# Anony-CFFM/CFFM

Measured on AMD Instinct MI355X. Metric: training examples/sec, frappe 10-field dim32; embedding-gather %HBM roofline, higher is better.
Workload: dtype f32; 1 GPU; frappe shape: synthetic libfm, 10 fields, 5382 features, inner/outer dim 32, batch 256 per GPU, selu, Adagrad lr 0.05, square_loss (README.md:28); global_batch=256, id_distribution=uniform, tables=replicated, parallelism=single

## Files before the change

### cffm_amd/csrc/common.hpp

```cpp
#pragma once
#include <hip/hip_runtime.h>
#include <stdint.h>

#include "../../include/cffm_hip.h"

#define CFFM_WAVE 64

#ifdef CFFM_PHASE_TIMERS
static __device__ unsigned long long cffm_phase_times[16];
static __device__ unsigned long long cffm_wg_times[2 * 1024];
static __device__ unsigned long long cffm_bwd_times[48];
#define PHASE_MARKB(i, wg) do { if ((wg) == 7 && threadIdx.x == 0) cffm_bwd_times[i] = wall_clock64(); } while (0)
#define PHASE_MARK(i) do { if (blockIdx.x == 7 && threadIdx.x == 0) cffm_phase_times[i] = wall_clock64(); } while (0)
#define PHASE_MARK2(i) do {} while (0)
#define PHASE_MARK3(i) do { if (CL && blockIdx.x == 7 && threadIdx.x == 0) cffm_phase_times[8 + (i)] = wall_clock64(); } while (0)
#else
#define PHASE_MARK(i) do {} while (0)
#define PHASE_MARK2(i) do {} while (0)
#define PHASE_MARK3(i) do {} while (0)
#define PHASE_MARKB(i, wg) do {} while (0)
#endif

typedef float f32x4 __attribute__((ext_vector_type(4)));
__device__ __forceinline__ int fused_c_off(int l, int c0, int c1, int D, int Pp) {
// ... 255 lines not shown

__device__ __forceinline__ float act_pos(float c, int act) {
    switch (act) {
        case CFFM_ACT_SELU: return CFFM_SELU_SCALE * c;
        case CFFM_ACT_GELU: return c * (0.5f * (1.f + erff(c * 0.70710678118654752440f)));
        default: return c;
    }
}

__device__ __forceinline__ float act_relu_grad(float c, int act) {
    return c > 0.f ? act_grad_f(c, act) : 0.f;
}

__device__ __forceinline__ void lds_barrier() {
    __builtin_amdgcn_fence(__ATOMIC_RELEASE, "workgroup", "local");
    __builtin_amdgcn_s_barrier();
    __builtin_amdgcn_fence(__ATOMIC_ACQUIRE, "workgroup", "local");
}

template <int CTRL, int ROW_MASK>
__device__ __forceinline__ float dpp_mov(float v, float identity) {
    return __builtin_bit_cast(float, __builtin_amdgcn_update_dpp(__builtin_bit_cast(int, identity), __builtin_bit_cast(int, v),
                                                                 CTRL, ROW_MASK, 0xf, false));
}
__device__ __forceinline__ float wave_sum(float v) {
    v += dpp_mov<0xB1, 0xf>(v, 0.f);
    v += dpp_mov<0x4E, 0xf>(v, 0.f);
    v += dpp_mov<0x141, 0xf>(v, 0.f);
    v += dpp_mov<0x140, 0xf>(v, 0.f);
    v += dpp_mov<0x142, 0xa>(v, 0.f);
    v += dpp_mov<0x143, 0xc>(v, 0.f);
    return __builtin_bit_cast(float, __builtin_amdgcn_readlane(__builtin_bit_cast(int, v), 63));
}
__device__ __forceinline__ float wave_max(float v) {
    const float ninf = -INFINITY;
    v = fmaxf(v, dpp_mov<0xB1, 0xf>(v, ninf));
    v = fmaxf(v, dpp_mov<0x4E, 0xf>(v, ninf));
    v = fmaxf(v, dpp_mov<0x141, 0xf>(v, ninf));
    v = fmaxf(v, dpp_mov<0x140, 0xf>(v, ninf));
    v = fmaxf(v, dpp_mov<0x142, 0xa>(v, ninf));
    v = fmaxf(v, dpp_mov<0x143, 0xc>(v, ninf));
    return __builtin_bit_cast(float, __builtin_amdgcn_readlane(__builtin_bit_cast(int, v), 63));
}

template <bool SIXTEEN>
__device__ __forceinline__ float row_group_sum(float v) {
    v += dpp_mov<0xB1, 0xf>(v, 0.f);
    v += dpp_mov<0x4E, 0xf>(v, 0.f);
    v += dpp_mov<0x141, 0xf>(v, 0.f);
    if (SIXTEEN) v += dpp_mov<0x140, 0xf>(v, 0.f);
    return v;
}

__device__ __forceinline__ float block_sum(float v, float* red) {
    v = wave_sum(v);
    const int w = threadIdx.x >> 6, nw = blockDim.x >> 6;
    __syncthreads();
    if ((threadIdx.x & 63) == 0) red[w] = v;
    __syncthreads();
    float t = 0.f;
    for (int i = 0; i < nw; ++i) t += red[i];
    return t;
}

__device__ __forceinline__ void build_pair_lut(uint32_t* lut, int F, int Pp) {
    for (int i = threadIdx.x; i < F; i += blockDim.x) {
        int base = i * (2 * F - i - 1) / 2;
        for (int j = i + 1; j < F; ++j) lut[base + j - i - 1] = (uint32_t)i | ((uint32_t)j << 16);
    }
    const int P = F * (F - 1) / 2;
    for (int p = P + threadIdx.x; p < Pp; p += blockDim.x) lut[p] = 0u;
}

__device__ __forceinline__ int fast_div(int n, float inv_d) { return (int)(((float)n + 0.5f) * inv_d); }

__device__ __forceinline__ f32x4 mfma16(float a, float b, f32x4 c) {
    return __builtin_amdgcn_mfma_f32_16x16x4f32(a, b, c, 0, 0, 0);
}
```

### cffm_amd/csrc/conv.hip

```cpp
#include <cstdlib>
#include <cstring>

#include "internal.hpp"

#include <type_traits>

#include <stdlib.h>
#include "inner_body.hpp"
#include "head_body.hpp"
#include "sort_body.hpp"

#define KSTEP 32
#define WG_KM 64

__device__ __forceinline__ int64_t xcd_tile(int64_t per_xcd) {
    const int64_t id = blockIdx.x;
    return (id & 7) * per_xcd + (id >> 3);
}
__host__ __device__ static inline int64_t xcd_per(int64_t tiles) { return (tiles + 7) / 8; }

struct RowPos { int b, y, x; };
__device__ __forceinline__ RowPos row_pos(int64_t m, int lgSo) {
    RowPos p;
    const int So = 1 << lgSo;
// ... 1550 lines not shown
    int early_off, es_off;
};


__device__ __forceinline__ unsigned rank_key_id(int raw, int M) { return min((unsigned)raw, (unsigned)M); }
template <int NW, int F_ = 0>
__device__ __forceinline__ void rank_keys_body(const int32_t* __restrict__ ids, int n, int b, int F_rt, int M,
                                               unsigned long long* __restrict__ out, char* smem) {
    constexpr int MAXF = F_ ? F_ : RANK_MAXF;
    const int F = F_ ? F_ : F_rt;
    float* cnt = reinterpret_cast<float*>(smem);
    const int tid = threadIdx.x, lane = tid & 63, wave = tid >> 6;
    unsigned long long mine[MAXF];
#pragma unroll
    for (int f = 0; f < MAXF; ++f) {
        const int slot = b * F + (f < F ? f : 0);
        mine[f] = f < F ? (((unsigned long long)rank_key_id(ids[slot], M) << 32) | (unsigned)slot) : 0ull;
    }
    int c[MAXF];
#pragma unroll
    for (int f = 0; f < MAXF; ++f) c[f] = 0;
    constexpr int GRP = 8;
    for (int j0 = tid; j0 < n; j0 += 64 * NW * GRP) {
        unsigned idj[GRP];
#pragma unroll
        for (int u = 0; u < GRP; ++u) {
            const int j = j0 + 64 * NW * u;
            idj[u] = rank_key_id(ids[j < n ? j : n - 1], M);
        }
#pragma unroll
        for (int u = 0; u < GRP; ++u) {
            const int j = j0 + 64 * NW * u;
            const unsigned long long kj = j < n ? (((unsigned long long)idj[u] << 32) | (unsigned)j) : ~0ull;
#pragma unroll
            for (int f = 0; f < MAXF; ++f) c[f] += kj < mine[f] ? 1 : 0;
        }
    }
#pragma unroll
    for (int f = 0; f < MAXF; ++f) {
        const float t = wave_sum((float)c[f]);
        if (lane == 0) cnt[wave * RANK_MAXF + f] = t;
    }
    __syncthreads();
    if (tid < F) {
        float c = cnt[tid];
#pragma unroll
        for (int w = 1; w < NW; ++w) c += cnt[w * RANK_MAXF + tid];
        const int rank = (int)c;
        const int slot = b * F + tid;
        out[rank] = ((unsigned long long)rank_key_id(ids[slot], M) << 32) | (unsigned)slot;
    }
    __syncthreads();
}

template <int N, int NTH>
struct ParkFilter {
    float4 w[N];
    float4* dst;
    int n4;
    __device__ __forceinline__ void fetch(const float4* src, float4* dst_, int n4_) {
        dst = dst_; n4 = src != nullptr ? n4_ : 0;
#pragma unroll
        for (int ii = 0; ii < N; ++ii) {
            const int i = threadIdx.x + NTH * ii;
            w[ii] = i < n4 ? src[i] : make_float4(0.f, 0.f, 0.f, 0.f);
        }
    }
    __device__ __forceinline__ void operator()() const {
#pragma unroll
        for (int ii = 0; ii < N; ++ii) {
            const int i = threadIdx.x + NTH * ii;
            if (i < n4) dst[i] = w[ii];
        }
    }
};

template <int N> using IntC = std::integral_constant<int, N>;
#define CV(x) decltype(x)::value
template <int L0, int L1, class Fn>
__device__ __forceinline__ void static_for(Fn&& fn) {
    if constexpr (L0 < L1) { fn(IntC<L0>()); static_for<L0 + 1, L1>(fn); }
}

template <int NT, int G, int ACT, int LGSO = -1>
__device__ __forceinline__ void fused_layer_fwd(const ConvArgs& ca, int b, char* smem, const float* inL, float* outL) {
    const int lgSo = LGSO >= 0 ? LGSO : ca.lgSo;
    const int64_t rows = 1ll << (2 * lgSo), m_lo = (int64_t)b * rows, m_hi = m_lo + rows;
    if (rows >= 64) {
        for (int64_t m0 = m_lo; m0 < m_hi; m0 += 64) {
            if (m0 > m_lo) lds_barrier();
            conv_fwd_taps_body<NT, 4 / G, false, G, ACT, LGSO>(ca, m0, m_hi, smem, inL, outL, m_lo);
        }
    } else if (rows >= 32) {
        conv_fwd_taps_body<NT, (G >= 2 ? 1 : 2), false, G, ACT, LGSO>(ca, m_lo, m_hi, smem, inL, outL, m_lo);
    } else {
        conv_fwd_taps_body<NT, 1, false, G, ACT, LGSO>(ca, m_lo, m_hi, smem, inL, outL, m_lo);
    }
}

template <int NT, int NW, int ACT = -1, int F_ = 0, int K_ = 0, int D_ = 0>
__global__ __launch_bounds__(64 * NW) void fwd_all_kernel(FwdAllArgs fa) {
    constexpr int G = NW / 4, PP = NT * 16;
    constexpr bool CS = F_ != 0;
    constexpr FwdAllLds PL = fwd_all_lds_plan(CS ? F_ : 2, CS ? K_ : 4, CS ? D_ : 4, PP);
    static_assert(!CS || (F_ * (F_ - 1) / 2 + 15) / 16 * 16 == PP, "NT is the column tile count of F_ fields");
    static_assert(!CS || (PL.c0_off >= 0 && PL.early_fits), "the compiled shape keeps its activations in LDS and gathers early");
    extern __shared__ __attribute__((aligned(16))) char smem[];
    const int c0_off = CS ? PL.c0_off : fa.c0_off, c1_off = CS ? PL.c1_off : fa.c1_off, es_off = CS ? PL.es_off : fa.es_off;
    const int D = CS ? D_ : fa.inner.g.D;
    int live = fa.live;
    if (CS) { live = -1; for (int d = D_; d > 1; d >>= 1) ++live; }
    auto CL = [&](int l) -> float* {
        return c0_off >= 0 ? reinterpret_cast<float*>(smem + fused_c_off(l, c0_off, c1_off, D, PP)) : nullptr;
    };
    const bool lds_act = c0_off >= 0;
#ifdef CFFM_PHASE_TIMERS
    if (threadIdx.x == 0) cffm_wg_times[2 * blockIdx.x] = wall_clock64();
#endif
    auto example = [&](int b) __attribute__((always_inline)) {
        ParkFilter<(4 * PP * PP / 4 + 64 * NW - 1) / (64 * NW), 64 * NW> park;
        const bool early = fa.early_off > 0;
        park.fetch(early ? reinterpret_cast<const float4*>(fa.conv[0].W) : nullptr, reinterpret_cast<float4*>(smem), 4 * PP * PP / 4);
        char* smem_i = smem + (CS ? (early ? PL.t_off : 0) : fa.early_off);
        if (fa.rank_keys) rank_keys_body<NW, F_>(fa.ids, fa.n_rows, b, fa.inner.g.F, fa.inner.g.M, fa.keys_sorted, smem_i);
        PHASE_MARK(0);
        inner_fwd_body<ACT, decltype(park), F_, K_, D_>(fa.inner, b, smem_i, early ? reinterpret_cast<float*>(smem + es_off) : nullptr,
                                                        D + 1, park);
        if (lds_act) lds_barrier(); else __syncthreads();
// ... 5 lines not shown
                lds_barrier();
                PHASE_MARK(1 + l);
                fused_layer_fwd<NT, G, ACT, LGSO>(fa.conv[l], b, smem, CL(l - 1), CL(l));
            });
        } else {
            for (int l = 1; l < live; ++l) {
                if (lds_act) lds_barrier(); else __syncthreads();
                PHASE_MARK(1 + l);
                fused_layer_fwd<NT, G, ACT>(fa.conv[l], b, smem, CL(l - 1), CL(l));
            }
        }
        if (lds_act) lds_barrier(); else __syncthreads();
        PHASE_MARK(1 + live);
        head_fwd_body<NW, ACT, false, F_, D_>(fa.head, b, smem, lds_act, c0_off, c1_off);
        PHASE_MARK(2 + live);
    };
    if constexpr (CS) {
        static_assert(!CS || 4096 / (CS ? F_ : 1) <= 2 * 256, "two passes over a grid of 256 workgroups cover every accepted B");
        if ((int)blockIdx.x < fa.B) example((int)blockIdx.x);
        if (const int b = blockIdx.x + gridDim.x; b < fa.B) {
            __syncthreads();
            example(b);
        }
    } else {
        for (int b = blockIdx.x; b < fa.B; b += gridDim.x) {
            if (b != (int)blockIdx.x) __syncthreads();
            example(b);
        }
    }
#ifdef CFFM_PHASE_TIMERS
    if (threadIdx.x == 0) cffm_wg_times[2 * blockIdx.x + 1] = wall_clock64();
#endif
}

template <int NT, int F_, int D_, int NW, bool ONE = false>
__device__ __forceinline__ void conv0_fact_bwd_body(const DgradArgs& a, float* __restrict__ slabW, float* __restrict__ slabB,
                                                    int64_t slab_stride, char* smem, int wg, int nwg) {
    constexpr int PP = NT * 16, S = 16, NTH = 64 * NW, XQ = 16 / NW;
    const int F = F_ ? F_ : a.F, D = D_ ? D_ : a.D, Dp = D + 1, P = F_ ? F_ * (F_ - 1) / 2 : a.P, F2 = 2 * F;
    const int TP = S * PP + 16;
    float* Wl = reinterpret_cast<float*>(smem);
    float* T = Wl + 4 * PP * PP;
    float* part = T + 2 * F * TP;
    float* dEi = part + NW * 16 * 32;
    float* dEj = dEi + 32 * 16;
    float* bred = dEj + 32 * 16;
    float* rs = bred + NW * PP;
    float* Es = rs + 2 * F;
    const int tid = threadIdx.x, lane = tid & 63, wave = tid >> 6, r = lane & 15, kk = lane >> 4;
    float* sw = slabW + (int64_t)wg * slab_stride;
    float* sb = slabB + (int64_t)wg * slab_stride;
    PHASE_MARKB(12, wg);
    {
        const float4* wsrc = reinterpret_cast<const float4*>(a.W);
        for (int i = tid; i < 4 * PP * PP / 4; i += NTH) reinterpret_cast<float4*>(Wl)[i] = wsrc[i];
        for (int e = tid; e < 4 * (PP - P) * PP; e += NTH) {
            const int tap = e / ((PP - P) * PP), o = e - tap * ((PP - P) * PP);
            sw[(tap * PP + P) * PP + o] = 0.f;
        }
    }
    bool first = true;
    float bacc[NT];
#pragma unroll
    for (int nt = 0; nt < NT; ++nt) bacc[nt] = 0.f;

    for (int b = wg; b < a.B; b += nwg) {
        __syncthreads();
        {
            const float* e = a.Cprev + (int64_t)b * F * D;
            const float invD = 1.f / (float)D;
            for (int i = tid; i < F * D; i += NTH) {
                const int f = fast_div(i, invD), d = i - f * D;
                Es[f * Dp + d] = e[i];
            }
        }
        __syncthreads();
        const float* dCb = a.dC + (int64_t)b * S * S * PP;
        PHASE_MARKB(13, wg);
        for (int u = wave; u < 2 * (F - 1); u += NW) {
            const int i = u % (F - 1), dh = u / (F - 1);
            const int nj = F - 1 - i, K = 2 * nj, base = i * (2 * F - i - 1) / 2;
            f32x4 acc[NT];
#pragma unroll
            for (int nt = 0; nt < NT; ++nt) acc[nt] = (f32x4){0.f, 0.f, 0.f, 0.f};
            for (int k0 = 0; k0 < K; k0 += 4) {
                const int k = k0 + kk;
                const bool ok = k < K;
                const int dw = (ok && k >= nj) ? 1 : 0, jj = ok ? k - dw * nj : 0;
                const float av = ok ? Es[(i + 1 + jj) * Dp + 2 * r + dw] : 0.f;
                const float* wr = Wl + ((dh * 2 + dw) * PP + base + jj) * PP + r;
#pragma unroll
                for (int nt = 0; nt < NT; ++nt) acc[nt] = mfma16(av, ok ? wr[nt * 16] : 0.f, acc[nt]);
            }
            float* tp = T + (dh * F + i) * TP + r;
#pragma unroll
            for (int nt = 0; nt < NT; ++nt)
#pragma unroll
                for (int j = 0; j < 4; ++j) tp[(kk * 4 + j) * PP + nt * 16] = acc[nt][j];
        }
        for (int e = tid; e < 2 * S * PP; e += NTH) {
            const int dh = e / (S * PP), o = e - dh * (S * PP);
            T[(dh * F + F - 1) * TP + o] = 0.f;
        }
        __syncthreads();
        PHASE_MARKB(14, wg);
        {
            f32x4 acc[2] = {(f32x4){0.f, 0.f, 0.f, 0.f}, (f32x4){0.f, 0.f, 0.f, 0.f}};
            float4 av[XQ][NT];
#pragma unroll
            for (int q4 = 0; q4 < XQ; ++q4)
#pragma unroll
                for (int h = 0; h < NT; ++h)
                    av[q4][h] = *reinterpret_cast<const float4*>(dCb + ((int64_t)r * S + wave + NW * q4) * PP + 16 * h + 4 * kk);
#pragma unroll
            for (int q4 = 0; q4 < XQ; ++q4) {
                const int x = wave + NW * q4;
#pragma unroll
                for (int h = 0; h < NT; ++h) {
                    float4 bv[2];
#pragma unroll
                    for (int ct = 0; ct < 2; ++ct) {
                        const int n = ct * 16 + r;
                        bv[ct] = n < F2 ? *reinterpret_cast<const float4*>(T + n * TP + x * PP + 16 * h + 4 * kk)
                                        : make_float4(0.f, 0.f, 0.f, 0.f);
                    }
#pragma unroll
                    for (int ct = 0; ct < 2; ++ct) {
// ... 421 lines not shown
    constexpr int PP = NT * 16, UNR = 4, NTH = 256 * HALVES;
    float* Bs = reinterpret_cast<float*>(smem);
    uint32_t* lut = reinterpret_cast<uint32_t*>(Bs + WGT_SUB * PP);
    float* Es = reinterpret_cast<float*>(lut + (GEN ? PP : 0));
    const int tid = tid_in >= 0 ? tid_in : (int)threadIdx.x, lane = tid & 63, wid = tid >> 6, tap = wid & 3, half = wid >> 2;
    const int r = lane & 15, kk = lane >> 4;
    const int So = 1 << a.lgSo, Sin = 2 * So, P = a.P, Dp = a.D + 1, S2 = So * So, dh = tap >> 1, dw = tap & 1;
    const int n_ex_max = GEN ? WGT_SUB / S2 + 2 : 0;
    f32x4* red = reinterpret_cast<f32x4*>(Es + (GEN ? (n_ex_max * a.F * Dp + 7) / 4 * 4 : 0));
    const int64_t rows_per_slab = ((a.Mtot + nslab - 1) / nslab + 3) / 4 * 4;
    const int64_t m_lo = m_lo_o >= 0 ? m_lo_o : slab * rows_per_slab;
    const int64_t m_hi = m_lo_o >= 0 ? m_hi_o : min(a.Mtot, m_lo + rows_per_slab);

    f32x4 acc[NT][NT];
#pragma unroll
    for (int i = 0; i < NT; ++i)
#pragma unroll
        for (int q = 0; q < NT; ++q) acc[i][q] = (f32x4){0.f, 0.f, 0.f, 0.f};
    float bs[NT];
#pragma unroll
    for (int q = 0; q < NT; ++q) bs[q] = 0.f;
    int fi[NT], fj[NT];
    if (GEN) {
        build_pair_lut(lut, a.F, PP);
        __syncthreads();
#pragma unroll
        for (int i = 0; i < NT; ++i) { const uint32_t ij = lut[i * 16 + r]; fi[i] = (ij & 0xffff) * Dp; fj[i] = (ij >> 16) * Dp; }
    }

    bool done_small = false;
    if constexpr (!GEN && HALVES == 1 && NT <= 4) {
        if (m_hi - m_lo <= 16 * UNR) {
            done_small = true;
            const int dbgw = (a.lgSo == 3 && m_lo_o < 0) ? slab : -1;
            PHASE_MARKB(32, dbgw);
            const int nrow = (int)max((int64_t)0, m_hi - m_lo), nk = (nrow + 3) / 4;
            float av[4][UNR][NT];
#pragma unroll
            for (int g = 0; g < 4; ++g)
                if (g * UNR < nk) {
#pragma unroll
                    for (int u = 0; u < UNR; ++u) {
                        int64_t m = m_lo + 4 * (g * UNR + u) + kk;
                        if (g * UNR + u >= nk || m >= a.Mtot) m = a.Mtot - 1;
                        const RowPos rp = row_pos(m, a.lgSo);
                        const float* arow = a.in + (((int64_t)rp.b * Sin + 2 * rp.y + dh) * Sin + 2 * rp.x + dw) * PP + r;
#pragma unroll
                        for (int i = 0; i < NT; ++i) av[g][u][i] = arow[16 * i];
                    }
                }
            __syncthreads();
            {
                const float4* src = reinterpret_cast<const float4*>(a.dC + m_lo * PP);
                for (int e = tid; e < nrow * (PP / 4); e += NTH) reinterpret_cast<float4*>(Bs)[e] = src[e];
                for (int e = nrow * (PP / 4) + tid; e < 4 * nk * (PP / 4); e += NTH)
                    reinterpret_cast<float4*>(Bs)[e] = make_float4(0.f, 0.f, 0.f, 0.f);
            }
            __syncthreads();
            PHASE_MARKB(33, dbgw);
#pragma unroll
            for (int g = 0; g < 4; ++g)
                if (g * UNR < nk) {
#pragma unroll
                    for (int u = 0; u < UNR; ++u)
                        if (g * UNR + u < nk) {
                            float bv[NT];
#pragma unroll
                            for (int q = 0; q < NT; ++q) bv[q] = Bs[(4 * (g * UNR + u) + kk) * PP + q * 16 + r];
#pragma unroll
                            for (int q = 0; q < NT; ++q) bs[q] += bv[q];
#pragma unroll
                            for (int i = 0; i < NT; ++i) {
                                const float x = act_pos(av[g][u][i], act);
#pragma unroll
                                for (int q = 0; q < NT; ++q) acc[i][q] = mfma16(x, bv[q], acc[i][q]);
                            }
                        }
                }
        }
    }
    PHASE_MARKB(34, (a.lgSo == 3 && m_lo_o < 0 && done_small) ? slab : -1);
    for (int64_t ms = m_lo; ms < m_hi && !done_small; ms += WGT_SUB) {
        const int nrow = (int)min((int64_t)WGT_SUB, m_hi - ms);
        const int b_lo = (int)(ms >> (2 * a.lgSo));
        __syncthreads();
        {
            const float4* src = reinterpret_cast<const float4*>(a.dC + ms * PP);
            for (int e = tid; e < nrow * (PP / 4); e += NTH) reinterpret_cast<float4*>(Bs)[e] = src[e];
            for (int e = nrow * (PP / 4) + tid; e < ((nrow + 3) / 4 * 4) * (PP / 4); e += NTH)
                reinterpret_cast<float4*>(Bs)[e] = make_float4(0.f, 0.f, 0.f, 0.f);
        }
        if (GEN) {
            const int b_hi = (int)((ms + nrow - 1) >> (2 * a.lgSo));
            stage_examples(Es, a.in, b_lo, b_hi - b_lo + 1, a.B, a.F, a.D, Dp);
        }
        __syncthreads();
        const int nk = (nrow + 3) / 4;
        int k0 = 0, k1 = nk;
        if (HALVES == 2) {
            const int mid = min(nk, ((nk + 1) / 2 + UNR - 1) / UNR * UNR);
            k0 = half == 0 ? 0 : mid;
            k1 = half == 0 ? mid : nk;
        }
        auto load_a = [&](int k, float (&av)[UNR][NT]) {
#pragma unroll
            for (int u = 0; u < UNR; ++u) {
                const int row = 4 * (k + u) + kk;
                int64_t m = ms + row;
                if (k + u >= k1 || m >= a.Mtot) m = a.Mtot - 1;
// ... 129 lines not shown

struct Conv01Args {
    DgradArgs d0;
    float *slabW0, *slabB0;
    int64_t stride0;
    DgradArgs d1;
    WgradArgs w1, w2, w3;
    int n2, n3;
};

template <int NT, int F_, int D_, int ACT>
__global__ __launch_bounds__(1024) void conv01_bwd_kernel(Conv01Args a) {
    extern __shared__ __attribute__((aligned(16))) char smem[];
    const int b = blockIdx.x, grp = __builtin_amdgcn_readfirstlane((int)(threadIdx.x >> 8)), ltid = threadIdx.x & 255;
    PHASE_MARKB(40, b);
    dgrad_taps_body<NT, 1, false, 4, ACT>(a.d1, b, smem, 0, -1, 4);
    PHASE_MARKB(41, b);
    {
        char* gsm = smem + (size_t)grp * (64 * NT * 16 * 4);
        const WgradArgs& w = grp == 0 ? a.w1 : (grp == 1 ? a.w2 : a.w3);
        const int nsl = grp == 0 ? (int)gridDim.x : (grp == 1 ? a.n2 : a.n3);
        const int slab = grp == 1 ? b - ((int)gridDim.x - a.n2) : b;
        const bool mine = grp < 3 && slab >= 0 && slab < nsl;
        int64_t m_lo = 0, m_hi = 0;
        if (mine) {
            const int64_t per = grp == 0 ? (1ll << (2 * w.lgSo)) : CFFM_TOP_SLAB_ROWS;
            m_lo = (int64_t)slab * per;
            m_hi = min(w.Mtot, m_lo + per);
            if (m_hi < m_lo) m_hi = m_lo;
        }
        wgrad_taps_body<NT, false, 1, ACT>(w, mine ? slab : 0, nsl, gsm, m_lo, m_hi, ltid, mine);
    }
    __syncthreads();
    PHASE_MARKB(42, b);
    conv0_fact_bwd_body<NT, F_, D_, 16, true>(a.d0, a.slabW0, a.slabB0, a.stride0, smem, b, (int)gridDim.x);
}

struct BwdTopArgs {
    HeadBwdArgs hb;
    DgradArgs d[2];
    WgradArgs w[2];
    int lgSo[2];
    int n_layers;
    int wgrad_here;
    InnerBwdArgs ib;
    int n_inner;
    int n_keys;
    const int32_t* rank_ids;
    unsigned long long* keys_sorted;
    int n_rows;
};

template <int NT, int ACT = -1>
__global__ __launch_bounds__(256) void bwd_top_kernel(BwdTopArgs a) {
    extern __shared__ __attribute__((aligned(16))) char smem[];
    __shared__ float dh1s[CFFM_HEAD_UNITS];
    __shared__ float dt1s[1024];
    __shared__ float red[4];
    const int bid = blockIdx.x;
#ifdef CFFM_PHASE_TIMERS
    if (threadIdx.x == 0) cffm_wg_times[2 * blockIdx.x] = wall_clock64();
#endif
    if (bid < a.n_inner) {
        PHASE_MARKB(36, bid);
        const float L = head_bwd_loss(a.hb, false, red);
        __syncthreads();
        PHASE_MARKB(37, bid);
        if (a.rank_ids != nullptr && a.n_keys == 0) {
            for (int b = bid; b < a.hb.B; b += a.n_inner) rank_keys_body<4>(a.rank_ids, a.n_rows, b, a.hb.g.F, a.hb.g.M, a.keys_sorted, smem);
        }
        PHASE_MARKB(38, bid);
        inner_bwd_body<ACT, true>(a.ib, bid, a.n_inner, smem, L);
        PHASE_MARKB(39, bid);
#ifdef CFFM_PHASE_TIMERS
        if (threadIdx.x == 0) cffm_wg_times[2 * blockIdx.x + 1] = wall_clock64();
#endif
        return;
    }
    if (bid < a.n_inner + a.n_keys) {
        for (int b = bid - a.n_inner; b < a.hb.B; b += a.n_keys) rank_keys_body<4>(a.rank_ids, a.n_rows, b, a.hb.g.F, a.hb.g.M, a.keys_sorted, smem);
#ifdef CFFM_PHASE_TIMERS
        if (threadIdx.x == 0) cffm_wg_times[2 * blockIdx.x + 1] = wall_clock64();
#endif
        return;
    }
    const int b = bid - a.n_inner - a.n_keys;
    PHASE_MARKB(0, b);
    HeadBwdState st;
    head_bwd_begin(a.hb, b, st);
    PHASE_MARKB(1, b);
    const float L = head_bwd_loss(a.hb, b == 0, red);
    PHASE_MARKB(2, b);
    if (b < a.hb.B)
        head_bwd_example<ACT>(a.hb, b, st, b, head_dout(a.hb.loss, a.hb.out[b], a.hb.y[b], 1.f / (float)a.hb.Bg, L), dh1s, dt1s);
    PHASE_MARKB(3, b);
    head_bwd_end(a.hb, b, st);
    PHASE_MARKB(4, b);
    for (int t = 0; t < a.n_layers; ++t) {
        __syncthreads();
        const int64_t rows = 1ll << (2 * a.lgSo[t]);
        const int64_t m_lo = (int64_t)b * rows, m_hi = b < a.hb.B ? m_lo + rows : m_lo;
        if (a.wgrad_here) wgrad_taps_body<NT, false, 1, ACT>(a.w[t], b, (int)gridDim.x - a.n_inner - a.n_keys, smem, m_lo, m_hi);
        PHASE_MARKB(5 + 2 * t, b);
        for (int64_t m0 = m_lo; m0 < m_hi; m0 += 16) dgrad_taps_body<NT, 1, false, 1, ACT>(a.d[t], 0, smem, m0, m_hi);
        PHASE_MARKB(6 + 2 * t, b);
    }
#ifdef CFFM_PHASE_TIMERS
    if (threadIdx.x == 0) cffm_wg_times[2 * blockIdx.x + 1] = wall_clock64();
#endif
}

template <int... Vs, class Go>
static int with_int(int v, Go&& go) {
    int rc = CFFM_ERR_UNSUPPORTED;
    (void)((v == Vs ? (rc = go(IntC<Vs>()), true) : false) || ...);
    return rc;
}
#define NT4 1, 2, 3, 4
#define NT68 6, 8
template <class... P, class... A>
static int launch(void (*kernel)(P...), dim3 grid, dim3 block, size_t lds, hipStream_t st, const A&... args) {
    int rc = set_lds(kernel, lds);
    if (rc) return rc;
    hipLaunchKernelGGL(kernel, grid, block, lds, st, args...);
    CFFM_CHECK_LAUNCH();
// ... 1498 lines not shown
```

### cffm_amd/csrc/head_body.hpp

```cpp
#pragma once
#include "common.hpp"

struct HeadArgs {
    Geo g;
    int B;
    const float* Eo;
    const float* fb;
    const float* inner_out;
    const float* C[CFFM_MAX_LAYERS];
    const float *d1_w, *d1_b, *d2_w, *d2_b, *att_W, *att_b, *lin_w, *lin_b, *bias;
    const float* y;
    float *t1, *h1, *att, *out, *sqerr;
    int loss, inner_conv, outer_conv;
    int s0_ready = 0;
    const float* pool[CFFM_MAX_LAYERS] = {};
    int pool_np[CFFM_MAX_LAYERS] = {};
};

__device__ __forceinline__ float loss_term(float out_raw, float y, int loss, float* out_eval) {
    switch (loss) {
        case CFFM_LOSS_MAE: *out_eval = out_raw; return fabsf(y - out_raw);
        case CFFM_LOSS_SQUARE_L2: *out_eval = out_raw; return 0.5f * (y - out_raw) * (y - out_raw);
        case CFFM_LOSS_LOG: {
            const float s = 1.f / (1.f + expf(-out_raw));
// ... 184 lines not shown
        out += o;
        out += sc[1];
        out += biasv;
        float ev = out;
        if (a.y) a.sqerr[b] = loss_term(out, yv, a.loss, &ev);
        else if (a.loss == CFFM_LOSS_LOG) ev = 1.f / (1.f + expf(-out));
        a.out[b] = ev;
    }
}

struct HeadBwdArgs {
    Geo g;
    int B;
    int64_t Bg;
    const float *fb, *t1, *h1, *att, *out, *y, *Ctop;
    const float *d1_w, *d2_w, *att_W, *lin_w;
    float* scalars;
    const float* sqerr;
    float* loss_out;
    float *dout, *dt1, *dfb, *dCtop;
    float *s_attW, *s_attb, *s_bias, *s_d1w, *s_d1b, *s_d2w, *s_d2b, *s_linw, *s_linb;
    int64_t stride_front, stride_back;
    int64_t front_len, back_len;
    int loss, outer_conv;
    int unscaled;
};

struct HeadBwdState {
    float g_d2w, g_d1b, g_d2b, g_bias, g_linw, g_linb, g_attb;
    bool first;
};

__device__ __forceinline__ void head_bwd_begin(const HeadBwdArgs& a, int slab, HeadBwdState& st) {
    const int tid = threadIdx.x;
    float* s_attW = a.s_attW + (int64_t)slab * a.stride_front;
    float* s_d1w = a.s_d1w + (int64_t)slab * a.stride_back;
    for (int64_t e = tid; e < a.front_len; e += 256) s_attW[e] = 0.f;
    for (int64_t e = tid; e < a.back_len; e += 256) s_d1w[e] = 0.f;
    st.g_d2w = st.g_d1b = st.g_d2b = st.g_bias = st.g_linw = st.g_linb = st.g_attb = 0.f;
    st.first = true;
    __syncthreads();
}

__device__ __forceinline__ float head_bwd_loss(const HeadBwdArgs& a, bool publisher, float* red) {
    const int tid = threadIdx.x;
    float sum = 0.f, hybrid_log = 0.f;
    if (a.loss == CFFM_LOSS_HYBRID) {
        float p_sq = 0.f, p_log = 0.f;
        for (int i = tid; i < a.B; i += 256) {
            const float o = a.out[i], yy = a.y[i];
            p_sq += 0.5f * (yy - o) * (yy - o);
            p_log -= yy * logf(o + 1e-7f) + (1.f - yy) * logf(1.f - o + 1e-7f);
        }
        sum = block_sum(p_sq, red);
        __syncthreads();
        hybrid_log = block_sum(p_log, red);
        __syncthreads();
    } else if (a.unscaled) {
        sum = 0.f;
    } else if (a.sqerr) {
        float part = 0.f;
        for (int i = tid; i < a.B; i += 256) part += a.sqerr[i];
        sum = block_sum(part, red);
        __syncthreads();
    } else {
        sum = a.scalars[3];
    }
    const float invB = 1.f / (float)a.Bg;
    float L;
    if (a.loss == CFFM_LOSS_SQUARE_RMSE) L = a.unscaled ? 1.f : sqrtf(sum * invB + 1e-10f);
    else if (a.loss == CFFM_LOSS_SQUARE_L2) L = sum;
    else if (a.loss == CFFM_LOSS_HYBRID) L = 0.5f * sum + 0.5f * hybrid_log * invB;
    else L = sum * invB;
    if (publisher && tid == 0) {
        a.scalars[1] = L;
        if (a.sqerr) { a.scalars[0] = sum; a.scalars[3] = sum; }
        if (a.loss_out) a.loss_out[0] = L;
    }
    return L;
}

template <int ACTC = -1>
__device__ __forceinline__ void head_bwd_example(const HeadBwdArgs& a, int slab, HeadBwdState& st, int b, float d,
                                                 float* dh1s, float* dt1s) {
    const Geo& g = a.g;
    const int tid = threadIdx.x, lane = tid & 63, wave = tid >> 6;
    const int t1w = 2 * g.D - 2;
    float* s_attW = a.s_attW + (int64_t)slab * a.stride_front;
    float* s_d1w = a.s_d1w + (int64_t)slab * a.stride_back;
    const bool first = st.first;
    int off_top = 0;
    for (int i = 0; i < g.live; ++i) off_top += g.D >> i;
    if (tid == 0) { a.dout[b] = d; st.g_bias += d; }
    __syncthreads();
    if (a.outer_conv) {
        const float dd = d * g.beta_outer;
        if (tid < CFFM_HEAD_UNITS) {
            const float v = dd * a.d2_w[tid];
            dh1s[tid] = v;
            st.g_d2w += a.h1[(int64_t)b * CFFM_HEAD_UNITS + tid] * dd;
            st.g_d1b += v;
        }
        if (tid == 0) st.g_d2b += dd;
        __syncthreads();
        for (int k = tid; k < t1w; k += 256) {
            float s = 0.f;
            for (int q = 0; q < CFFM_HEAD_UNITS; ++q) s += dh1s[q] * a.d1_w[k * CFFM_HEAD_UNITS + q];
            dt1s[k] = s;
            a.dt1[(int64_t)b * t1w + k] = s;
        }
        for (int e = tid; e < t1w * CFFM_HEAD_UNITS; e += 256) {
            const int k = e / CFFM_HEAD_UNITS, q = e % CFFM_HEAD_UNITS;
            const float v = a.t1[(int64_t)b * t1w + k] * dh1s[q];
            s_d1w[e] = first ? v : s_d1w[e] + v;
        }
        __syncthreads();
        const int ntop = 4 * g.Pp;
        for (int e = tid; e < ntop; e += 256) {
            const int yy = e / (2 * g.Pp);
            const int64_t idx = (int64_t)b * ntop + e;
            a.dCtop[idx] = dt1s[off_top + yy] * act_relu_grad(a.Ctop[idx], ACTC >= 0 ? ACTC : g.act);
        }
    }
    if (wave == 0) {
        const float fbv = lane < g.F ? a.fb[(int64_t)b * g.F + lane] : 0.f;
        if (g.linear_att) {
            const float at = lane < g.F ? a.att[(int64_t)b * g.F + lane] : 0.f;
            const float dg = lane < g.F ? d * a.lin_w[lane] : 0.f;
            const float da = dg * fbv;
            const float sda = wave_sum(da * at);
            const float dz = at * (da - sda) / g.lamda_att;
            float dfbv = dg * at;
            for (int gI = 0; gI < g.F; ++gI) {
                const float dzg = __shfl(dz, gI, 64);
                if (lane < g.F) {
                    dfbv += dzg * a.att_W[lane * g.F + gI];
                    const float v = fbv * dzg;
                    s_attW[lane * g.F + gI] = first ? v : s_attW[lane * g.F + gI] + v;
                }
            }
            if (lane < g.F) a.dfb[(int64_t)b * g.F + lane] = dfbv;
            st.g_linw += fbv * at * d;
            st.g_attb += dz;
            if (lane == 0) st.g_linb += d;
        } else if (lane < g.F) {
            a.dfb[(int64_t)b * g.F + lane] = d;
        }
    }
    st.first = false;
}

__device__ __forceinline__ void head_bwd_end(const HeadBwdArgs& a, int slab, const HeadBwdState& st) {
    const int tid = threadIdx.x;
    const int64_t sof = (int64_t)slab * a.stride_front, sob = (int64_t)slab * a.stride_back;
    if (tid < CFFM_HEAD_UNITS) {
        a.s_d2w[sob + tid] = st.g_d2w;
        a.s_d1b[sob + tid] = st.g_d1b;
    }
    if (tid < a.g.F) {
        a.s_linw[sob + tid] = st.g_linw;
        a.s_attb[sof + tid] = st.g_attb;
    }
    if (tid == 0) {
        a.s_d2b[sob] = st.g_d2b;
        a.s_bias[sof] = st.g_bias;
        a.s_linb[sob] = st.g_linb;
    }
}
```

### cffm_amd/csrc/inner_body.hpp

```cpp
#pragma once
#include "common.hpp"

struct InnerUnit {
    float x0, x1, I0, I1, z0, z1, s0, s1, eix, eiy, ejx, ejy;
    int i, j;
};

__device__ __forceinline__ InnerUnit inner_unit(const float* E, const uint32_t* lut, int p, int t, int K,
                                                const float* cw, const float* cb, int act) {
    InnerUnit u;
    const uint32_t ij = lut[p];
    u.i = ij & 0xffff; u.j = ij >> 16;
    const float2 ei = *reinterpret_cast<const float2*>(&E[u.i * K + 2 * t]);
    const float2 ej = *reinterpret_cast<const float2*>(&E[u.j * K + 2 * t]);
    u.eix = ei.x; u.eiy = ei.y; u.ejx = ej.x; u.ejy = ej.y;
    u.I0 = ei.x * ej.x; u.I1 = ei.y * ej.y;
    u.x0 = act_f(u.I0, act); u.x1 = act_f(u.I1, act);
    u.z0 = u.x0 * cw[0] + u.x1 * cw[2] + cb[0];
    u.z1 = u.x0 * cw[1] + u.x1 * cw[3] + cb[1];
    const float mp = fmaxf(u.x0, u.x1);
    u.s0 = act_pos(fmaxf(u.z0, 0.f), act) + mp;
    u.s1 = act_pos(fmaxf(u.z1, 0.f), act) + mp;
    return u;
}
// ... 57 lines not shown
                reinterpret_cast<float4*>(fg.Eo + (int64_t)b * g.F * g.D)[j] = v;
                if (EoL != nullptr) {
                    float* e = EoL + f * EoLp + 4 * c;
                    e[0] = v.x; e[1] = v.y; e[2] = v.z; e[3] = v.w;
                }
            }
        }
        if (threadIdx.x < g.F) {
            const int raw = idb[threadIdx.x];
            const int id = raw < 0 ? 0 : (raw >= fg.M ? fg.M - 1 : raw);
            const int64_t slot = (int64_t)b * g.F + threadIdx.x;
            fg.fb[slot] = fg.fbias[id];
            fg.keys[slot] = ((unsigned long long)(unsigned)((raw < 0 || raw >= fg.M) ? fg.M : raw) << 32) | (unsigned long long)slot;
        }
    } else {
        mid();
        const float4* src = reinterpret_cast<const float4*>(Ei + (int64_t)b * g.F * g.K);
        for (int i = threadIdx.x; i < FK4; i += blockDim.x) reinterpret_cast<float4*>(E)[i] = src[i];
    }
    build_pair_lut(lut, g.F, g.Pp);
    float cw[4] = {cw_g[0], cw_g[1], cw_g[2], cw_g[3]};
    float cb[2] = {cb_g[0], cb_g[1]};
    const int K2 = g.K / 2, units = g.P * K2;
    const float2* wd2 = reinterpret_cast<const float2*>(wd);
    const float2 w2_first = (int)threadIdx.x < units ? wd2[threadIdx.x] : make_float2(0.f, 0.f);
    __syncthreads();
    const float invK2 = 1.f / (float)K2;
    float part = 0.f;
    for (int u = threadIdx.x; u < units; u += blockDim.x) {
        const int p = fast_div(u, invK2), t = u - p * K2;
        const InnerUnit v = inner_unit(E, lut, p, t, g.K, cw, cb, act);
        const float2 w2 = u == (int)threadIdx.x ? w2_first : wd2[u];
        part += v.s0 * w2.x + v.s1 * w2.y;
    }
    const float tot = block_sum(part, red);
    if (threadIdx.x == 0) inner_out[b] = tot + bd[0];
}

struct InnerBwdArgs {
    Geo g;
    int B;
    const float *Ei, *dout, *cw, *cb, *wd;
    const float *out, *y;
    int loss;
    float invB;
    float* dEi;
    float *slab_cw, *slab_cb, *slab_dw, *slab_db;
    int64_t slab_stride;
    const int32_t* idx = nullptr;
    int idxM = 0;
    int idxStride = 0;
};

template <int ACTC = -1, bool ONE = false>
__device__ __forceinline__ void inner_bwd_body(const InnerBwdArgs& a, int slab, int nslab, char* smem, float L = 1.f) {
    const Geo& g = a.g;
    const int act = ACTC >= 0 ? ACTC : g.act;
    const int B = a.B;
    const float* __restrict__ Ei = a.Ei; const float* __restrict__ dout = a.dout;
    const float* __restrict__ cw_g = a.cw; const float* __restrict__ cb_g = a.cb; const float* __restrict__ wd = a.wd;
    float* __restrict__ dEi = a.dEi;
    float* __restrict__ slab_cw = a.slab_cw + slab * a.slab_stride; float* __restrict__ slab_cb = a.slab_cb + slab * a.slab_stride;
    float* __restrict__ slab_dw = a.slab_dw + slab * a.slab_stride; float* __restrict__ slab_db = a.slab_db + slab * a.slab_stride;
    const int FK = g.F * g.K;
    float* E = reinterpret_cast<float*>(smem);
    float* dE = E + FK;
    uint32_t* lut = reinterpret_cast<uint32_t*>(dE + 4 * FK);
    float* red = reinterpret_cast<float*>(lut + g.Pp);
    const int wave = threadIdx.x >> 6;
    build_pair_lut(lut, g.F, g.Pp);
    if (threadIdx.x < 8) slab_cw[threadIdx.x] = 0.f;
    if (threadIdx.x < 4) slab_db[threadIdx.x] = 0.f;
    float cw[4] = {cw_g[0], cw_g[1], cw_g[2], cw_g[3]};
    float cb[2] = {cb_g[0], cb_g[1]};
    const int K2 = g.K / 2, units = g.P * K2;
    const float invK2 = 1.f / (float)K2;
    float gcw[4] = {0.f, 0.f, 0.f, 0.f}, gcb[2] = {0.f, 0.f}, gdb = 0.f;
    constexpr int UPRE = 4;
    const float2* wd2 = reinterpret_cast<const float2*>(wd);
    float2 w2p[UPRE];
#pragma unroll
    for (int k = 0; k < UPRE; ++k) {
        const int u = threadIdx.x + k * blockDim.x;
        w2p[k] = u < units ? wd2[u] : make_float2(0.f, 0.f);
    }
    bool first = true;
    for (int b = slab; b < B; b += nslab) {
        const float db = dout ? dout[b] : head_dout(a.loss, a.out[b], a.y[b], a.invB, L);
        __syncthreads();
        if (a.idx == nullptr) {
            const float4* src = reinterpret_cast<const float4*>(Ei + (int64_t)b * FK);
            for (int i = threadIdx.x; i < FK / 4; i += blockDim.x) reinterpret_cast<float4*>(E)[i] = src[i];
        } else {
            const int K4 = g.K >> 2;
            const float invK4 = 1.f / (float)K4;
            for (int i = threadIdx.x; i < FK / 4; i += blockDim.x) {
                const int f = fast_div(i, invK4), c = i - f * K4;
                reinterpret_cast<float4*>(E)[i] =
                    reinterpret_cast<const float4*>(row_ptr(Ei, a.idx, a.idxM, (int64_t)b * g.F + f, g.K, a.idxStride))[c];
            }
        }
        for (int i = threadIdx.x; i < 4 * FK; i += blockDim.x) dE[i] = 0.f;
        __syncthreads();
        float* myE = dE + wave * FK;
        auto unit_step = [&](int u, float2 w2) {
            const int p = fast_div(u, invK2), t = u - p * K2;
            const InnerUnit v = inner_unit(E, lut, p, t, g.K, cw, cb, act);
            const int64_t wi = (int64_t)p * g.K + 2 * t;
            float2 acc2 = first ? make_float2(0.f, 0.f) : *reinterpret_cast<float2*>(&slab_dw[wi]);
            acc2.x += v.s0 * db; acc2.y += v.s1 * db;
            *reinterpret_cast<float2*>(&slab_dw[wi]) = acc2;
            const float ds0 = db * w2.x, ds1 = db * w2.y;
            const float dz0 = ds0 * act_relu_grad(fmaxf(v.z0, 0.f), act);
            const float dz1 = ds1 * act_relu_grad(fmaxf(v.z1, 0.f), act);
            gcw[0] += dz0 * v.x0; gcw[1] += dz1 * v.x0; gcw[2] += dz0 * v.x1; gcw[3] += dz1 * v.x1;
            gcb[0] += dz0; gcb[1] += dz1;
            const float dmp = ds0 + ds1;
            const bool firstmax = v.x0 >= v.x1;
            const float dx0 = dz0 * cw[0] + dz1 * cw[1] + (firstmax ? dmp : 0.f);
            const float dx1 = dz0 * cw[2] + dz1 * cw[3] + (firstmax ? 0.f : dmp);
            const float dI0 = dx0 * act_grad_f(v.I0, act), dI1 = dx1 * act_grad_f(v.I1, act);
            atomicAdd(&myE[v.i * g.K + 2 * t], dI0 * v.ejx);
            atomicAdd(&myE[v.i * g.K + 2 * t + 1], dI1 * v.ejy);
            atomicAdd(&myE[v.j * g.K + 2 * t], dI0 * v.eix);
            atomicAdd(&myE[v.j * g.K + 2 * t + 1], dI1 * v.eiy);
        };
#pragma unroll
        for (int k = 0; k < UPRE; ++k) {
            const int u = threadIdx.x + k * blockDim.x;
            if (u < units) unit_step(u, w2p[k]);
        }
        for (int u = threadIdx.x + UPRE * blockDim.x; u < units; u += blockDim.x) unit_step(u, wd2[u]);
        if (threadIdx.x == 0) gdb += db;
        __syncthreads();
        for (int i = threadIdx.x; i < FK; i += blockDim.x)
            dEi[(int64_t)b * FK + i] = ((dE[i] + dE[FK + i]) + dE[2 * FK + i]) + dE[3 * FK + i];
        first = false;
        if constexpr (ONE) break;
    }
    if (first) {
        for (int64_t i = threadIdx.x; i < (int64_t)g.P * g.K; i += blockDim.x) slab_dw[i] = 0.f;
    }
    float r[7] = {gcw[0], gcw[1], gcw[2], gcw[3], gcb[0], gcb[1], gdb};
#pragma unroll
    for (int q = 0; q < 7; ++q) r[q] = wave_sum(r[q]);
    __syncthreads();
    if ((threadIdx.x & 63) == 0) {
#pragma unroll
        for (int q = 0; q < 7; ++q) dE[wave * 8 + q] = r[q];
    }
    __syncthreads();
    if (threadIdx.x == 0) {
        const int nw = blockDim.x >> 6;
#pragma unroll
        for (int q = 0; q < 7; ++q) {
            float t = 0.f;
            for (int w = 0; w < nw; ++w) t += dE[w * 8 + q];
            r[q] = t;
        }
        for (int q = 0; q < 4; ++q) slab_cw[q] = r[q];
        slab_cb[0] = r[4]; slab_cb[1] = r[5];
        slab_db[0] = r[6];
    }
}
```

Measured before the change: 2.981 million examples/s.

## Issue global loads early in backward kernels to hide latency behind loss reduction

Inner backward now prefetches the embedding row, out/y scalars and zeroes dE before computing the block-wide loss, passing the loss computation as a callback so the loads overlap it. Several copy loops are restructured to issue batches of loads before stores (loads_first, ParkFilter), attention-weight reads are batched in groups of 12, blockDim is replaced by a compile-time 256, and bwd_top_kernel gets an occupancy hint. The rank-key computation is removed from this kernel path, which risks changing behaviour if it is not done elsewhere; extra registers from the unrolled loads could also reduce occupancy.

```diff
diff --git a/cffm_amd/csrc/common.hpp b/cffm_amd/csrc/common.hpp
--- a/cffm_amd/csrc/common.hpp
+++ b/cffm_amd/csrc/common.hpp
@@ -331,9 +331,10 @@
     return v;
 }
 
+template <int NTH = 0>
 __device__ __forceinline__ float block_sum(float v, float* red) {
     v = wave_sum(v);
-    const int w = threadIdx.x >> 6, nw = blockDim.x >> 6;
+    const int w = threadIdx.x >> 6, nw = NTH ? NTH >> 6 : (int)blockDim.x >> 6;
     __syncthreads();
     if ((threadIdx.x & 63) == 0) red[w] = v;
     __syncthreads();
@@ -342,13 +343,15 @@
     return t;
 }
 
+template <int NTH = 0>
 __device__ __forceinline__ void build_pair_lut(uint32_t* lut, int F, int Pp) {
-    for (int i = threadIdx.x; i < F; i += blockDim.x) {
+    const int nth = NTH ? NTH : (int)blockDim.x;
+    for (int i = threadIdx.x; i < F; i += nth) {
         int base = i * (2 * F - i - 1) / 2;
         for (int j = i + 1; j < F; ++j) lut[base + j - i - 1] = (uint32_t)i | ((uint32_t)j << 16);
     }
     const int P = F * (F - 1) / 2;
-    for (int p = P + threadIdx.x; p < Pp; p += blockDim.x) lut[p] = 0u;
+    for (int p = P + threadIdx.x; p < Pp; p += nth) lut[p] = 0u;
 }
 
 __device__ __forceinline__ int fast_div(int n, float inv_d) { return (int)(((float)n + 0.5f) * inv_d); }
@@ -356,3 +359,43 @@
 __device__ __forceinline__ f32x4 mfma16(float a, float b, f32x4 c) {
     return __builtin_amdgcn_mfma_f32_16x16x4f32(a, b, c, 0, 0, 0);
 }
+
+
+template <int N, int NTH>
+struct ParkFilter {
+    float4 w[N];
+    float4* dst;
+    int n4;
+    __device__ __forceinline__ void fetch(const float4* src, float4* dst_, int n4_) {
+        dst = dst_; n4 = src != nullptr ? n4_ : 0;
+#pragma unroll
+        for (int ii = 0; ii < N; ++ii) {
+            const int i = threadIdx.x + NTH * ii;
+            w[ii] = i < n4 ? src[i] : make_float4(0.f, 0.f, 0.f, 0.f);
+        }
+    }
+    __device__ __forceinline__ void operator()() const {
+#pragma unroll
+        for (int ii = 0; ii < N; ++ii) {
+            const int i = threadIdx.x + NTH * ii;
+            if (i < n4) dst[i] = w[ii];
+        }
+    }
+};
+
+template <int U, int NTH, class T, class Load, class Use>
+__device__ __forceinline__ void loads_first(int tid, int n, Load&& load, Use&& use) {
+    for (int e0 = tid; e0 < n; e0 += U * NTH) {
+        T v[U];
+#pragma unroll
+        for (int u = 0; u < U; ++u) {
+            const int e = e0 + u * NTH;
+            if (e < n) v[u] = load(e);
+        }
+#pragma unroll
+        for (int u = 0; u < U; ++u) {
+            const int e = e0 + u * NTH;
+            if (e < n) use(e, v[u]);
+        }
+    }
+}
diff --git a/cffm_amd/csrc/conv.hip b/cffm_amd/csrc/conv.hip
--- a/cffm_amd/csrc/conv.hip
+++ b/cffm_amd/csrc/conv.hip
@@ -1626,28 +1626,6 @@
     }
     __syncthreads();
 }
-
-template <int N, int NTH>
-struct ParkFilter {
-    float4 w[N];
-    float4* dst;
-    int n4;
-    __device__ __forceinline__ void fetch(const float4* src, float4* dst_, int n4_) {
-        dst = dst_; n4 = src != nullptr ? n4_ : 0;
-#pragma unroll
-        for (int ii = 0; ii < N; ++ii) {
-            const int i = threadIdx.x + NTH * ii;
-            w[ii] = i < n4 ? src[i] : make_float4(0.f, 0.f, 0.f, 0.f);
-        }
-    }
-    __device__ __forceinline__ void operator()() const {
-#pragma unroll
-        for (int ii = 0; ii < N; ++ii) {
-            const int i = threadIdx.x + NTH * ii;
-            if (i < n4) dst[i] = w[ii];
-        }
-    }
-};
 
 template <int N> using IntC = std::integral_constant<int, N>;
 #define CV(x) decltype(x)::value
@@ -1759,8 +1737,9 @@
     float* sb = slabB + (int64_t)wg * slab_stride;
     PHASE_MARKB(12, wg);
     {
-        const float4* wsrc = reinterpret_cast<const float4*>(a.W);
-        for (int i = tid; i < 4 * PP * PP / 4; i += NTH) reinterpret_cast<float4*>(Wl)[i] = wsrc[i];
+        ParkFilter<(4 * PP * PP / 4 + NTH - 1) / NTH, NTH> park;
+        park.fetch(reinterpret_cast<const float4*>(a.W), reinterpret_cast<float4*>(Wl), 4 * PP * PP / 4);
+        park();
         for (int e = tid; e < 4 * (PP - P) * PP; e += NTH) {
             const int tap = e / ((PP - P) * PP), o = e - tap * ((PP - P) * PP);
             sw[(tap * PP + P) * PP + o] = 0.f;
@@ -1776,10 +1755,10 @@
         {
             const float* e = a.Cprev + (int64_t)b * F * D;
             const float invD = 1.f / (float)D;
-            for (int i = tid; i < F * D; i += NTH) {
+            loads_first<2, NTH, float>(tid, F * D, [&](int i) { return e[i]; }, [&](int i, float v) {
                 const int f = fast_div(i, invD), d = i - f * D;
-                Es[f * Dp + d] = e[i];
-            }
+                Es[f * Dp + d] = v;
+            });
         }
         __syncthreads();
         const float* dCb = a.dC + (int64_t)b * S * S * PP;
@@ -2307,9 +2286,11 @@
             __syncthreads();
             {
                 const float4* src = reinterpret_cast<const float4*>(a.dC + m_lo * PP);
-                for (int e = tid; e < nrow * (PP / 4); e += NTH) reinterpret_cast<float4*>(Bs)[e] = src[e];
-                for (int e = nrow * (PP / 4) + tid; e < 4 * nk * (PP / 4); e += NTH)
-                    reinterpret_cast<float4*>(Bs)[e] = make_float4(0.f, 0.f, 0.f, 0.f);
+                float4* Bs4 = reinterpret_cast<float4*>(Bs);
+                const int nld = nrow * (PP / 4);
+                loads_first<NT, NTH, float4>(tid, 4 * nk * (PP / 4),
+                    [&](int e) { return e < nld ? src[e] : make_float4(0.f, 0.f, 0.f, 0.f); },
+                    [&](int e, const float4& v) { Bs4[e] = v; });
             }
             __syncthreads();
             PHASE_MARKB(33, dbgw);
@@ -2545,7 +2526,7 @@
 };
 
 template <int NT, int ACT = -1>
-__global__ __launch_bounds__(256) void bwd_top_kernel(BwdTopArgs a) {
+__global__ __launch_bounds__(256, (NT <= 3 ? 3 : 1)) void bwd_top_kernel(BwdTopArgs a) {
     extern __shared__ __attribute__((aligned(16))) char smem[];
     __shared__ float dh1s[CFFM_HEAD_UNITS];
     __shared__ float dt1s[1024];
@@ -2556,14 +2537,13 @@
 #endif
     if (bid < a.n_inner) {
         PHASE_MARKB(36, bid);
-        const float L = head_bwd_loss(a.hb, false, red);
-        __syncthreads();
-        PHASE_MARKB(37, bid);
-        if (a.rank_ids != nullptr && a.n_keys == 0) {
-            for (int b = bid; b < a.hb.B; b += a.n_inner) rank_keys_body<4>(a.rank_ids, a.n_rows, b, a.hb.g.F, a.hb.g.M, a.keys_sorted, smem);
-        }
-        PHASE_MARKB(38, bid);
-        inner_bwd_body<ACT, true>(a.ib, bid, a.n_inner, smem, L);
+        inner_bwd_body<ACT, true>(a.ib, bid, a.n_inner, smem, [&]() __attribute__((always_inline)) {
+            const float L = head_bwd_loss(a.hb, false, red);
+            __syncthreads();
+            PHASE_MARKB(37, bid);
+            PHASE_MARKB(38, bid);
+            return L;
+        });
         PHASE_MARKB(39, bid);
 #ifdef CFFM_PHASE_TIMERS
         if (threadIdx.x == 0) cffm_wg_times[2 * blockIdx.x + 1] = wall_clock64();
diff --git a/cffm_amd/csrc/head_body.hpp b/cffm_amd/csrc/head_body.hpp
--- a/cffm_amd/csrc/head_body.hpp
+++ b/cffm_amd/csrc/head_body.hpp
@@ -260,16 +260,16 @@
             p_sq += 0.5f * (yy - o) * (yy - o);
             p_log -= yy * logf(o + 1e-7f) + (1.f - yy) * logf(1.f - o + 1e-7f);
         }
-        sum = block_sum(p_sq, red);
-        __syncthreads();
-        hybrid_log = block_sum(p_log, red);
+        sum = block_sum<256>(p_sq, red);
+        __syncthreads();
+        hybrid_log = block_sum<256>(p_log, red);
         __syncthreads();
     } else if (a.unscaled) {
         sum = 0.f;
     } else if (a.sqerr) {
         float part = 0.f;
         for (int i = tid; i < a.B; i += 256) part += a.sqerr[i];
-        sum = block_sum(part, red);
+        sum = block_sum<256>(part, red);
         __syncthreads();
     } else {
         sum = a.scalars[3];
@@ -317,10 +317,15 @@
             dt1s[k] = s;
             a.dt1[(int64_t)b * t1w + k] = s;
         }
-        for (int e = tid; e < t1w * CFFM_HEAD_UNITS; e += 256) {
-            const int k = e / CFFM_HEAD_UNITS, q = e % CFFM_HEAD_UNITS;
-            const float v = a.t1[(int64_t)b * t1w + k] * dh1s[q];
-            s_d1w[e] = first ? v : s_d1w[e] + v;
+        {
+            static_assert(256 % CFFM_HEAD_UNITS == 0, "a thread's q does not change from trip to trip");
+            const float* t1b = a.t1 + (int64_t)b * t1w;
+            loads_first<8, 256, float>(tid, t1w * CFFM_HEAD_UNITS,
+                [&](int e) { return t1b[e / CFFM_HEAD_UNITS]; },
+                [&](int e, float t) {
+                    const float v = t * dh1s[e % CFFM_HEAD_UNITS];
+                    s_d1w[e] = first ? v : s_d1w[e] + v;
+                });
         }
         __syncthreads();
         const int ntop = 4 * g.Pp;
@@ -339,12 +344,26 @@
             const float sda = wave_sum(da * at);
             const float dz = at * (da - sda) / g.lamda_att;
             float dfbv = dg * at;
-            for (int gI = 0; gI < g.F; ++gI) {
-                const float dzg = __shfl(dz, gI, 64);
+            constexpr int AW = 12;
+            for (int g0 = 0; g0 < g.F; g0 += AW) {
+                float aw[AW], dzg[AW];
+#pragma unroll
+                for (int u = 0; u < AW; ++u)
+                    if (lane < g.F && g0 + u < g.F) aw[u] = a.att_W[lane * g.F + g0 + u];
+#pragma unroll
+                for (int u = 0; u < AW; ++u) dzg[u] = __shfl(dz, (g0 + u) & 63, 64);
                 if (lane < g.F) {
-                    dfbv += dzg * a.att_W[lane * g.F + gI];
-                    const float v = fbv * dzg;
-                    s_attW[lane * g.F + gI] = first ? v : s_attW[lane * g.F + gI] + v;
+#pragma unroll
+                    for (int u = 0; u < AW; ++u)
+                        if (g0 + u < g.F) dfbv += dzg[u] * aw[u];
+#pragma unroll
+                    for (int u = 0; u < AW; ++u) {
+                        const int gI = g0 + u;
+                        if (gI < g.F) {
+                            const float v = fbv * dzg[u];
+                            s_attW[lane * g.F + gI] = first ? v : s_attW[lane * g.F + gI] + v;
+                        }
+                    }
                 }
             }
             if (lane < g.F) a.dfb[(int64_t)b * g.F + lane] = dfbv;
diff --git a/cffm_amd/csrc/inner_body.hpp b/cffm_amd/csrc/inner_body.hpp
--- a/cffm_amd/csrc/inner_body.hpp
+++ b/cffm_amd/csrc/inner_body.hpp
@@ -133,8 +133,10 @@
     int idxStride = 0;
 };
 
-template <int ACTC = -1, bool ONE = false>
-__device__ __forceinline__ void inner_bwd_body(const InnerBwdArgs& a, int slab, int nslab, char* smem, float L = 1.f) {
+struct InnerNoLoss { __device__ __forceinline__ float operator()() const { return 1.f; } };
+template <int ACTC = -1, bool ONE = false, class BeforeLoop = InnerNoLoss>
+__device__ __forceinline__ void inner_bwd_body(const InnerBwdArgs& a, int slab, int nslab, char* smem, BeforeLoop&& before_loop = BeforeLoop()) {
+    constexpr int NTH = 256;
     const Geo& g = a.g;
     const int act = ACTC >= 0 ? ACTC : g.act;
     const int B = a.B;
@@ -149,7 +151,7 @@
     uint32_t* lut = reinterpret_cast<uint32_t*>(dE + 4 * FK);
     float* red = reinterpret_cast<float*>(lut + g.Pp);
     const int wave = threadIdx.x >> 6;
-    build_pair_lut(lut, g.F, g.Pp);
+    build_pair_lut<NTH>(lut, g.F, g.Pp);
     if (threadIdx.x < 8) slab_cw[threadIdx.x] = 0.f;
     if (threadIdx.x < 4) slab_db[threadIdx.x] = 0.f;
     float cw[4] = {cw_g[0], cw_g[1], cw_g[2], cw_g[3]};
@@ -162,26 +164,38 @@
     float2 w2p[UPRE];
 #pragma unroll
     for (int k = 0; k < UPRE; ++k) {
-        const int u = threadIdx.x + k * blockDim.x;
+        const int u = threadIdx.x + k * NTH;
         w2p[k] = u < units ? wd2[u] : make_float2(0.f, 0.f);
     }
+    ParkFilter<1, NTH> erows;
+    float out1 = 0.f, y1 = 0.f;
+    const bool pre = ONE && a.idx == nullptr && slab < B;
+    if constexpr (ONE) {
+        erows.fetch(pre ? reinterpret_cast<const float4*>(Ei + (int64_t)slab * FK) : nullptr, reinterpret_cast<float4*>(E), FK / 4);
+        if (!dout && slab < B) { out1 = a.out[slab]; y1 = a.y[slab]; }
+        for (int i = threadIdx.x; i < 4 * FK; i += NTH) dE[i] = 0.f;
+    }
+    const float L = before_loop();
     bool first = true;
     for (int b = slab; b < B; b += nslab) {
-        const float db = dout ? dout[b] : head_dout(a.loss, a.out[b], a.y[b], a.invB, L);
+        const float db = dout ? dout[b] : (ONE ? head_dout(a.loss, out1, y1, a.invB, L) : head_dout(a.loss, a.out[b], a.y[b], a.invB, L));
         __syncthreads();
         if (a.idx == nullptr) {
             const float4* src = reinterpret_cast<const float4*>(Ei + (int64_t)b * FK);
-            for (int i = threadIdx.x; i < FK / 4; i += blockDim.x) reinterpret_cast<float4*>(E)[i] = src[i];
+            if constexpr (ONE) erows();
+            for (int i = threadIdx.x + (ONE ? NTH : 0); i < FK / 4; i += NTH) reinterpret_cast<float4*>(E)[i] = src[i];
         } else {
             const int K4 = g.K >> 2;
             const float invK4 = 1.f / (float)K4;
-            for (int i = threadIdx.x; i < FK / 4; i += blockDim.x) {
+            for (int i = threadIdx.x; i < FK / 4; i += NTH) {
                 const int f = fast_div(i, invK4), c = i - f * K4;
                 reinterpret_cast<float4*>(E)[i] =
                     reinterpret_cast<const float4*>(row_ptr(Ei, a.idx, a.idxM, (int64_t)b * g.F + f, g.K, a.idxStride))[c];
             }
         }
-        for (int i = threadIdx.x; i < 4 * FK; i += blockDim.x) dE[i] = 0.f;
+        if constexpr (!ONE) {
+            for (int i = threadIdx.x; i < 4 * FK; i += NTH) dE[i] = 0.f;
+        }
         __syncthreads();
         float* myE = dE + wave * FK;
         auto unit_step = [&](int u, float2 w2) {
@@ -208,19 +222,20 @@
         };
 #pragma unroll
         for (int k = 0; k < UPRE; ++k) {
-            const int u = threadIdx.x + k * blockDim.x;
+            const int u = threadIdx.x + k * NTH;
             if (u < units) unit_step(u, w2p[k]);
         }
-        for (int u = threadIdx.x + UPRE * blockDim.x; u < units; u += blockDim.x) unit_step(u, wd2[u]);
+#pragma unroll 1
+        for (int u = threadIdx.x + UPRE * NTH; u < units; u += NTH) unit_step(u, wd2[u]);
         if (threadIdx.x == 0) gdb += db;
         __syncthreads();
-        for (int i = threadIdx.x; i < FK; i += blockDim.x)
+        for (int i = threadIdx.x; i < FK; i += NTH)
             dEi[(int64_t)b * FK + i] = ((dE[i] + dE[FK + i]) + dE[2 * FK + i]) + dE[3 * FK + i];
         first = false;
         if constexpr (ONE) break;
     }
     if (first) {
-        for (int64_t i = threadIdx.x; i < (int64_t)g.P * g.K; i += blockDim.x) slab_dw[i] = 0.f;
+        for (int64_t i = threadIdx.x; i < (int64_t)g.P * g.K; i += NTH) slab_dw[i] = 0.f;
     }
     float r[7] = {gcw[0], gcw[1], gcw[2], gcw[3], gcb[0], gcb[1], gdb};
 #pragma unroll
@@ -232,7 +247,7 @@
     }
     __syncthreads();
     if (threadIdx.x == 0) {
-        const int nw = blockDim.x >> 6;
+        const int nw = NTH >> 6;
 #pragma unroll
         for (int q = 0; q < 7; ++q) {
             float t = 0.f;
```

Result: faster. 3.022 million examples/s (median of 6 runs) (+1.4%).
